# stdstu12/YUME

Hardware: AMD Instinct MI355X
Metric: denoise-steps/sec (Yume-5B 720P, 33-frame latent) (higher is better)
Workload: dtype bf16; 1 GPU; Yume-5B-720P random-init, 33-frame 704x1280 clip (latent 48x13x44x80, FramePack lfz=8, L=9460), ODE Euler steps of a 50-step shift-7 schedule, no CFG, one chain per GPU; num_layers=30, parallelism=dp1 (independent chains, replicated weights)

## Files before the change

yume_amd/csrc/gemm_f8.hpp:

```cpp
#pragma once
#include "gemm_w4.hpp"

namespace gemm_f8 {
using namespace gemm_core;

typedef __attribute__((ext_vector_type(8))) int i32x8;

constexpr int F8_BK = 128;
constexpr int F8_NTHR = 256;
constexpr int F8_OPER = 256 * F8_BK;
constexpr int F8_BUF = 2 * F8_OPER;
constexpr int F8_LDS = 2 * F8_BUF;

struct F8Args {
    const unsigned char* A; int64_t lda; const float* sa;
    const unsigned char* W; int64_t ldw; const float* sw;
    const unsigned char* ea; int64_t ldea;
    unsigned char* eo; int64_t ldeo;
};

constexpr int EPI_MX_GELU = YUME_EPI_MX_GELU;

__device__ __forceinline__ void f8_stage(const unsigned char* const (&ga)[8], const unsigned char* const (&gw)[8], int koff, char* buf, int wave) {
#pragma unroll
    for (int j = 0; j < 8; ++j)
        __builtin_amdgcn_global_load_lds((gbl_cvoid*)(ga[j] + koff), (lds_void*)(buf + j * 4096 + wave * 1024), 16, 0, 0);
#pragma unroll
    for (int j = 0; j < 8; ++j)
        __builtin_amdgcn_global_load_lds((gbl_cvoid*)(gw[j] + koff), (lds_void*)(buf + F8_OPER + j * 4096 + wave * 1024), 16, 0, 0);
}

__device__ __forceinline__ i32x8 f8_frag(const char* oper, int row, int lane) {
    const int q = lane >> 4;
    const char* rp = oper + row * F8_BK;
    const u32x4 lo = *reinterpret_cast<const u32x4*>(rp + ((((2 * q) ^ row) & 7) << 4));
    const u32x4 hi = *reinterpret_cast<const u32x4*>(rp + ((((2 * q + 1) ^ row) & 7) << 4));
    return i32x8{(int)lo[0], (int)lo[1], (int)lo[2], (int)lo[3], (int)hi[0], (int)hi[1], (int)hi[2], (int)hi[3]};
}

template <class Col>
__device__ __forceinline__ void f8_epilogue_vt(const f32x4 (&acc)[8][8], const float (&sa)[8], Col col, const Problem& p, const Epilogue& e, int m0,
                                               int n0, char* smem) {
    const int lane = threadIdx.x & 63;
    const int wave = __builtin_amdgcn_readfirstlane(threadIdx.x >> 6);
    const int wr = wave >> 1, wc = wave & 1;
    const int l15 = lane & 15, l4 = lane >> 4;
    const bool odd = (l15 & 1) != 0;
    const int x0 = 4 * l4 + 2 * (l15 & 1);
    const unsigned vbase = (unsigned)((wc * 128 + x0) * 512 + ((l15 >> 1) & 3) * 4);
    const unsigned lx = (unsigned)((x0 | (l15 >> 3)) << 4);
    __syncthreads();
#pragma unroll
    for (int j = 0; j < 8; ++j) {
        f32x4 sw, b;
        col(j, sw, b);
        const unsigned jb = vbase + (unsigned)(16 * j * 512) + (unsigned)((wr ^ (j & 1)) << 8);
#pragma unroll
        for (int i = 0; i < 8; ++i) {
            const f32x4 v = (acc[i][j] * sa[i]) * sw + b;
            const unsigned p01 = pack_bf16x2(v[0], v[1]), p23 = pack_bf16x2(v[2], v[3]);
            const unsigned got = (unsigned)__builtin_amdgcn_update_dpp(0, (int)(odd ? p01 : p23), 0xB1, 0xf, 0xf, false);
            const unsigned keep = odd ? p23 : p01;
            const unsigned lo = odd ? got : keep, hi = odd ? keep : got;
            *reinterpret_cast<unsigned*>(smem + jb + (lx ^ (unsigned)((2 * i) << 4))) = (lo & 0xffffu) | (hi << 16);
            *reinterpret_cast<unsigned*>(smem + jb + 512u + (lx ^ (unsigned)((2 * i + 1) << 4))) = (lo >> 16) | (hi & 0xffff0000u);
        }
    }
    __syncthreads();
    gemm_w4::w4_store_image(smem, e.outT + (int64_t)(n0 - e.n_split) * e.ldt, e.ldt, 0, min(256, p.N - n0), m0, min(256, p.M - m0));
}

template <int EPI, bool MX = false>
__device__ __forceinline__ void f8_epilogue(const f32x4 (&acc)[8][8], const Problem& p, const F8Args& f, const Epilogue& e, int m0, int n0, char* smem) {
    const int lane = threadIdx.x & 63;
    const int wave = __builtin_amdgcn_readfirstlane(threadIdx.x >> 6);
    const int wr = wave >> 1, wc = wave & 1;
    const int l15 = lane & 15, l4 = lane >> 4;
    float sa[8];
#pragma unroll
    for (int i = 0; i < 8; ++i) sa[i] = MX ? 1.0f : f.sa[min(m0 + wr * 128 + 16 * i + l15, p.M - 1)];
    auto col = [&](int j, f32x4& sw, f32x4& b) {
        const int n = n0 + wc * 128 + 16 * j + 4 * l4;
        sw = n < p.N ? *reinterpret_cast<const f32x4*>(f.sw + n) : f32x4{1.f, 1.f, 1.f, 1.f};
        b = (e.bias && n < p.N) ? *reinterpret_cast<const f32x4*>(e.bias + n) : f32x4{0.f, 0.f, 0.f, 0.f};
    };
    if constexpr (EPI == YUME_EPI_BF16_SPLITT) {
        if (n0 >= e.n_split) {
            f8_epilogue_vt(acc, sa, col, p, e, m0, n0, smem);
            return;
        }
    }
    constexpr int EPI_RM = EPI == YUME_EPI_BF16_SPLITT ? YUME_EPI_BF16 : EPI;
    constexpr bool BF16_OUT = EPI_RM == YUME_EPI_BF16 || EPI_RM == YUME_EPI_BF16_GELU;
    if (BF16_OUT && (e.ldo % 8) == 0) {
        const gemm_w4::ImageOff io = gemm_w4::w4_image_offsets(wr, wc, l15, l4);
        __syncthreads();
#pragma unroll
        for (int j = 0; j < 8; ++j) {
            f32x4 sw, b;
            col(j, sw, b);
#pragma unroll
            for (int i = 0; i < 8; ++i) {
                const f32x4 v = gemm_w4::w4_act<EPI>((acc[i][j] * sa[i]) * sw + b);
                u32x2 o;
                o[0] = pack_bf16x2(v[0], v[1]);
                o[1] = pack_bf16x2(v[2], v[3]);
                *reinterpret_cast<u32x2*>(smem + ((i & 1) ? io.o[j] : io.e[j]) + i * 8192) = o;
            }
        }
        __syncthreads();
        gemm_w4::w4_store_image(smem, reinterpret_cast<unsigned short*>(e.out), e.ldo, m0, min(256, p.M - m0), n0, min(256, p.N - n0));
        return;
    }
    Epilogue e0 = e;
    e0.bias = nullptr;
#pragma unroll
    for (int j = 0; j < 8; ++j) {
        f32x4 sw, b;
        col(j, sw, b);
#pragma unroll
        for (int i = 0; i < 8; ++i) {
            const int m = m0 + wr * 128 + 16 * i + l15, n = n0 + wc * 128 + 16 * j + 4 * l4;
            if (m < p.M && n < p.N) store_row4<EPI_RM>((acc[i][j] * sa[i]) * sw + b, m, n, p, e0);
        }
    }
}

__device__ __forceinline__ void f8_epilogue_mx_gelu(const f32x4 (&acc)[8][8], const Problem& p, const F8Args& f, const Epilogue& e, int m0, int n0) {
    const int lane = threadIdx.x & 63;
    const int wave = __builtin_amdgcn_readfirstlane(threadIdx.x >> 6);
    const int wr = wave >> 1, wc = wave & 1;
    const int l15 = lane & 15, l4 = lane >> 4;
    float sa[8];
#pragma unroll
    for (int i = 0; i < 8; ++i) sa[i] = f.sa[min(m0 + wr * 128 + 16 * i + l15, p.M - 1)];
    unsigned char* const qo = reinterpret_cast<unsigned char*>(e.out);
#pragma unroll
    for (int jj = 0; jj < 4; ++jj) {
        const int nb = n0 + wc * 128 + 32 * jj;
        const bool in_n = nb < p.N;
        f32x4 sw[2], b[2];
#pragma unroll
        for (int h = 0; h < 2; ++h) {
            const int n = nb + 16 * h + 4 * l4;
            sw[h] = in_n ? *reinterpret_cast<const f32x4*>(f.sw + n) : f32x4{1.f, 1.f, 1.f, 1.f};
            b[h] = (e.bias && in_n) ? *reinterpret_cast<const f32x4*>(e.bias + n) : f32x4{0.f, 0.f, 0.f, 0.f};
        }
#pragma unroll
        for (int i = 0; i < 8; ++i) {
            const int m = m0 + wr * 128 + 16 * i + l15;
            f32x4 v[2];
            float am = 0.f;
#pragma unroll
            for (int h = 0; h < 2; ++h) {
                v[h] = gemm_w4::w4_act<YUME_EPI_BF16_GELU>((acc[i][2 * jj + h] * sa[i]) * sw[h] + b[h]);
#pragma unroll
                for (int c = 0; c < 4; ++c) am = fmaxf(am, fabsf(v[h][c]));
            }
            am = fmaxf(am, __shfl_xor(am, 16, 64));
            am = fmaxf(am, __shfl_xor(am, 32, 64));
            const unsigned bits = __float_as_uint(am);
            const int E = (int)(bits >> 23);
            int byte = E - 8 + ((bits & 0x7fffffu) > 0x600000u ? 1 : 0);
            byte = am > 0.f ? max(byte, 0) : 127;
            const float mult = __uint_as_float((unsigned)(254 - byte) << 23);
            if (m < p.M && in_n) {
#pragma unroll
                for (int h = 0; h < 2; ++h) {
                    float t[4];
#pragma unroll
                    for (int c = 0; c < 4; ++c) t[c] = fminf(fmaxf(v[h][c] * mult, -448.0f), 448.0f);
                    int w = __builtin_amdgcn_cvt_pk_fp8_f32(t[0], t[1], 0, false);
                    w = __builtin_amdgcn_cvt_pk_fp8_f32(t[2], t[3], w, true);
                    *reinterpret_cast<int*>(qo + (int64_t)m * e.ldo + nb + 16 * h + 4 * l4) = w;
                }
                if (l4 == 0) f.eo[(int64_t)m * f.ldeo + (nb >> 5)] = (unsigned char)byte;
            }
        }
    }
}

__device__ __forceinline__ i32x8 f8_frag_mx(const char* oper, int row, int lane) {
    const int q = lane >> 4;
    const char* rp = oper + row * F8_BK;
    const u32x4 lo = *reinterpret_cast<const u32x4*>(rp + (((q ^ row) & 7) << 4));
    const u32x4 hi = *reinterpret_cast<const u32x4*>(rp + ((((4 + q) ^ row) & 7) << 4));
    return i32x8{(int)lo[0], (int)lo[1], (int)lo[2], (int)lo[3], (int)hi[0], (int)hi[1], (int)hi[2], (int)hi[3]};
}

__device__ __forceinline__ void f8_mx_scales_load(const unsigned char* const (&ge)[8], int g, u32x4 (&raw)[8]) {
#pragma unroll
    for (int i = 0; i < 8; ++i) raw[i] = *reinterpret_cast<const u32x4*>(ge[i] + 16 * g);
}
__device__ __forceinline__ void f8_mx_scales_pack(const u32x4 (&raw)[8], int lane, unsigned (&pk)[8]) {
    const int sh = 8 * (lane >> 4);
#pragma unroll
    for (int i = 0; i < 8; ++i)
        pk[i] = ((raw[i][0] >> sh) & 0xffu) | (((raw[i][1] >> sh) & 0xffu) << 8) | (((raw[i][2] >> sh) & 0xffu) << 16) | ((raw[i][3] >> sh) << 24 & 0xff000000u);
}

template <int EPI>
__global__ __launch_bounds__(F8_NTHR, 1) void gemm_f8_mx_kernel(Problem p, F8Args f, Epilogue e) {
    __shared__ __attribute__((aligned(16))) char smem[F8_LDS];
    const int tid = threadIdx.x;
    const int lane = tid & 63;
    const int wave = __builtin_amdgcn_readfirstlane(tid >> 6);
    const int wr = wave >> 1, wc = wave & 1;
    int start, count, m0, n0;
    xcd_chunk(p.tiles_m * p.tiles_n, blockIdx.x & 7, start, count);
    tile_origin(p, start + (blockIdx.x >> 3), m0, n0);

    const unsigned char* ga[8];
    const unsigned char* gw[8];
    const unsigned char* ge[8];
    {
        const int rl = 8 * wave + (lane >> 3);
#pragma unroll
        for (int j = 0; j < 8; ++j) {
            const int r = 32 * j + rl;
            const int ch = ((lane & 7) ^ (r & 7)) << 4;
            ga[j] = f.A + (int64_t)min(m0 + r, p.M - 1) * f.lda + ch;
            gw[j] = f.W + (int64_t)min(n0 + r, p.N - 1) * f.ldw + ch;
        }
#pragma unroll
        for (int i = 0; i < 8; ++i) ge[i] = f.ea + (int64_t)min(m0 + wr * 128 + 16 * i + (lane & 15), p.M - 1) * f.ldea;
    }
    f32x4 acc[8][8];
#pragma unroll
    for (int i = 0; i < 8; ++i)
#pragma unroll
        for (int j = 0; j < 8; ++j) acc[i][j] = f32x4{0.f, 0.f, 0.f, 0.f};

    const int nk = p.K / F8_BK;
    u32x4 raw[8];
    unsigned pk[8], pkn[8];
    f8_mx_scales_load(ge, 0, raw);
    f8_stage(ga, gw, 0, smem, wave);
    f8_mx_scales_pack(raw, lane, pk);
#pragma unroll
    for (int i = 0; i < 8; ++i) pkn[i] = pk[i];
    int cur = 0;
    for (int kt = 0; kt < nk; ++kt) {
        asm volatile("s_waitcnt vmcnt(0)" ::: "memory");
        __syncthreads();
        const int t = kt & 3;
        if (t == 3) f8_mx_scales_pack(raw, lane, pkn);
        if (t == 2 && kt + 2 < nk) f8_mx_scales_load(ge, (kt >> 2) + 1, raw);
        if (kt + 1 < nk) f8_stage(ga, gw, (kt + 1) * F8_BK, smem + (cur ^ 1) * F8_BUF, wave);
        const char* At = smem + cur * F8_BUF;
        const char* Wt = At + F8_OPER;
        i32x8 a[8];
        int sc[8];
#pragma unroll
        for (int i = 0; i < 8; ++i) {
            a[i] = f8_frag_mx(At, wr * 128 + 16 * i + (lane & 15), lane);
            sc[i] = (int)(pk[i] >> (8 * t));
        }
#pragma unroll
        for (int j = 0; j < 8; ++j) {
            const i32x8 w = f8_frag_mx(Wt, wc * 128 + 16 * j + (lane & 15), lane);
#pragma unroll
            for (int i = 0; i < 8; ++i)
                acc[i][j] = __builtin_amdgcn_mfma_scale_f32_16x16x128_f8f6f4(w, a[i], acc[i][j], 0, 0, 0, 0x7f7f7f7f, 0, sc[i]);
        }
        if (t == 3) {
#pragma unroll
            for (int i = 0; i < 8; ++i) pk[i] = pkn[i];
        }
        cur ^= 1;
    }
    f8_epilogue<EPI, true>(acc, p, f, e, m0, n0, smem);
}

template <int EPI>
__global__ __launch_bounds__(F8_NTHR, 1) void gemm_f8_kernel(Problem p, F8Args f, Epilogue e) {
    __shared__ __attribute__((aligned(16))) char smem[F8_LDS];
    const int tid = threadIdx.x;
    const int lane = tid & 63;
    const int wave = __builtin_amdgcn_readfirstlane(tid >> 6);
    const int wr = wave >> 1, wc = wave & 1;
    int start, count, m0, n0;
    xcd_chunk(p.tiles_m * p.tiles_n, blockIdx.x & 7, start, count);
    tile_origin(p, start + (blockIdx.x >> 3), m0, n0);

    const unsigned char* ga[8];
    const unsigned char* gw[8];
    {
        const int rl = 8 * wave + (lane >> 3);
#pragma unroll
        for (int j = 0; j < 8; ++j) {
            const int r = 32 * j + rl;
            const int ch = ((lane & 7) ^ (r & 7)) << 4;
            ga[j] = f.A + (int64_t)min(m0 + r, p.M - 1) * f.lda + ch;
            gw[j] = f.W + (int64_t)min(n0 + r, p.N - 1) * f.ldw + ch;
        }
    }
    f32x4 acc[8][8];
#pragma unroll
    for (int i = 0; i < 8; ++i)
#pragma unroll
        for (int j = 0; j < 8; ++j) acc[i][j] = f32x4{0.f, 0.f, 0.f, 0.f};

    const int nk = p.K / F8_BK;
    f8_stage(ga, gw, 0, smem, wave);
    int cur = 0;
    for (int kt = 0; kt < nk; ++kt) {
        asm volatile("s_waitcnt vmcnt(0)" ::: "memory");
        __syncthreads();
        if (kt + 1 < nk) f8_stage(ga, gw, (kt + 1) * F8_BK, smem + (cur ^ 1) * F8_BUF, wave);
        const char* At = smem + cur * F8_BUF;
        const char* Wt = At + F8_OPER;
        i32x8 a[8];
#pragma unroll
        for (int i = 0; i < 8; ++i) a[i] = f8_frag(At, wr * 128 + 16 * i + (lane & 15), lane);
#pragma unroll
        for (int j = 0; j < 8; ++j) {
            const i32x8 w = f8_frag(Wt, wc * 128 + 16 * j + (lane & 15), lane);
#pragma unroll
            for (int i = 0; i < 8; ++i)
                acc[i][j] = __builtin_amdgcn_mfma_scale_f32_16x16x128_f8f6f4(w, a[i], acc[i][j], 0, 0, 0, 0x7f7f7f7f, 0, 0x7f7f7f7f);
        }
        cur ^= 1;
    }
    if constexpr (EPI == EPI_MX_GELU) f8_epilogue_mx_gelu(acc, p, f, e, m0, n0);
    else f8_epilogue<EPI>(acc, p, f, e, m0, n0, smem);
}

inline int launch_f8(int epi, Problem p, const F8Args& f, const Epilogue& e, hipStream_t st) {
    p.tiles_m = (p.M + 255) / 256;
    p.tiles_n = (p.N + 255) / 256;
    p.group_m = g_group_m;
    const dim3 grid((unsigned)(p.tiles_m * p.tiles_n)), block(F8_NTHR);
    switch (epi) {
        case YUME_EPI_BF16_GELU: hipLaunchKernelGGL(gemm_f8_kernel<YUME_EPI_BF16_GELU>, grid, block, 0, st, p, f, e); break;
        case YUME_EPI_F32: hipLaunchKernelGGL(gemm_f8_kernel<YUME_EPI_F32>, grid, block, 0, st, p, f, e); break;
        case YUME_EPI_RESID: hipLaunchKernelGGL(gemm_f8_kernel<YUME_EPI_RESID>, grid, block, 0, st, p, f, e); break;
        case EPI_MX_GELU: hipLaunchKernelGGL(gemm_f8_kernel<EPI_MX_GELU>, grid, block, 0, st, p, f, e); break;
        case YUME_EPI_BF16_SPLITT: hipLaunchKernelGGL(gemm_f8_kernel<YUME_EPI_BF16_SPLITT>, grid, block, 0, st, p, f, e); break;
        default: hipLaunchKernelGGL(gemm_f8_kernel<YUME_EPI_BF16>, grid, block, 0, st, p, f, e); break;
    }
    YUME_CHECK_LAUNCH("gemm_f8");
    return YUME_OK;
}

inline int launch_f8_mx(int epi, Problem p, const F8Args& f, const Epilogue& e, hipStream_t st) {
    p.tiles_m = (p.M + 255) / 256;
    p.tiles_n = (p.N + 255) / 256;
    p.group_m = g_group_m;
    const dim3 grid((unsigned)(p.tiles_m * p.tiles_n)), block(F8_NTHR);
    if (epi == YUME_EPI_RESID) hipLaunchKernelGGL(gemm_f8_mx_kernel<YUME_EPI_RESID>, grid, block, 0, st, p, f, e);
    else hipLaunchKernelGGL(gemm_f8_mx_kernel<YUME_EPI_F32>, grid, block, 0, st, p, f, e);
    YUME_CHECK_LAUNCH("gemm_f8_mx");
    return YUME_OK;
}

}
```

Baseline: 10.46 denoise-steps/sec.

## Interleave FP8 GEMM LDS reads, global loads and MFMAs with sched group barriers

Adds a scheduled main-loop variant for the FP8 and MX-FP8 GEMM kernels. It uses sched_group_barrier to interleave LDS fragment reads and next-tile global loads between the 64 MFMAs of each K step, and peels the last iteration so it does no staging. The goal is to hide memory latency behind matrix work instead of letting the compiler cluster loads. The variant is on by default for the GELU, RESID and MX-GELU epilogues and selectable through an environment variable, at the cost of doubled template instantiations and more register pressure.

```diff
diff --git a/yume_amd/csrc/gemm_f8.hpp b/yume_amd/csrc/gemm_f8.hpp
--- a/yume_amd/csrc/gemm_f8.hpp
+++ b/yume_amd/csrc/gemm_f8.hpp
@@ -199,7 +199,41 @@
         pk[i] = ((raw[i][0] >> sh) & 0xffu) | (((raw[i][1] >> sh) & 0xffu) << 8) | (((raw[i][2] >> sh) & 0xffu) << 16) | ((raw[i][3] >> sh) << 24 & 0xff000000u);
 }
 
-template <int EPI>
+constexpr int F8_SG_MFMA = 0x8, F8_SG_VMEM = 0x10, F8_SG_DS_READ = 0x100;
+template <bool MX, bool STAGE>
+__device__ __forceinline__ void f8_tile_sched(f32x4 (&acc)[8][8], const char* __restrict__ At, const unsigned char* const (&ga)[8],
+                                              const unsigned char* const (&gw)[8], int koff, char* __restrict__ nbuf, int wave, int wr, int wc, int lane,
+                                              const int (&sc)[8]) {
+    __builtin_amdgcn_sched_barrier(0);
+    if constexpr (STAGE) f8_stage(ga, gw, koff, nbuf, wave);
+    const char* Wt = At + F8_OPER;
+    i32x8 a[8];
+#pragma unroll
+    for (int i = 0; i < 8; ++i) a[i] = MX ? f8_frag_mx(At, wr * 128 + 16 * i + (lane & 15), lane) : f8_frag(At, wr * 128 + 16 * i + (lane & 15), lane);
+#pragma unroll
+    for (int j = 0; j < 8; ++j) {
+        const i32x8 w = MX ? f8_frag_mx(Wt, wc * 128 + 16 * j + (lane & 15), lane) : f8_frag(Wt, wc * 128 + 16 * j + (lane & 15), lane);
+#pragma unroll
+        for (int i = 0; i < 8; ++i)
+            acc[i][j] = __builtin_amdgcn_mfma_scale_f32_16x16x128_f8f6f4(w, a[i], acc[i][j], 0, 0, 0, 0x7f7f7f7f, 0, MX ? sc[i] : 0x7f7f7f7f);
+    }
+    __builtin_amdgcn_sched_group_barrier(F8_SG_DS_READ, 8, 0);
+#pragma unroll
+    for (int m = 0; m < 64; ++m) {
+        __builtin_amdgcn_sched_group_barrier(F8_SG_MFMA, 1, 0);
+        if (m < 5 || m == 5 || (m >= 8 && m < 56 && (m & 7) == 3)) __builtin_amdgcn_sched_group_barrier(F8_SG_DS_READ, 2, 0);
+        if (STAGE && m < 32 && (m & 1)) __builtin_amdgcn_sched_group_barrier(F8_SG_VMEM, 1, 0);
+    }
+    __builtin_amdgcn_sched_barrier(0);
+    if constexpr (!STAGE) {
+#pragma unroll
+        for (int i = 0; i < 8; ++i)
+#pragma unroll
+            for (int j = 0; j < 8; ++j) asm volatile("" : "+a"(acc[i][j]));
+    }
+}
+
+template <int EPI, int LOOP>
 __global__ __launch_bounds__(F8_NTHR, 1) void gemm_f8_mx_kernel(Problem p, F8Args f, Epilogue e) {
     __shared__ __attribute__((aligned(16))) char smem[F8_LDS];
     const int tid = threadIdx.x;
@@ -240,6 +274,25 @@
 #pragma unroll
     for (int i = 0; i < 8; ++i) pkn[i] = pk[i];
     int cur = 0;
+    if constexpr (LOOP == 1) {
+        int sc[8];
+        for (int kt = 0; kt + 1 < nk; ++kt) {
+            asm volatile("s_waitcnt vmcnt(0)" ::: "memory");
+            __syncthreads();
+            const int t = kt & 3;
+#pragma unroll
+            for (int i = 0; i < 8; ++i) sc[i] = (int)(pk[i] >> (8 * t));
+            if (t == 3) f8_mx_scales_pack(raw, lane, pk);
+            if (t == 2 && kt + 2 < nk) f8_mx_scales_load(ge, (kt >> 2) + 1, raw);
+            f8_tile_sched<true, true>(acc, smem + cur * F8_BUF, ga, gw, (kt + 1) * F8_BK, smem + (cur ^ 1) * F8_BUF, wave, wr, wc, lane, sc);
+            cur ^= 1;
+        }
+        asm volatile("s_waitcnt vmcnt(0)" ::: "memory");
+        __syncthreads();
+#pragma unroll
+        for (int i = 0; i < 8; ++i) sc[i] = (int)(pk[i] >> (8 * ((nk - 1) & 3)));
+        f8_tile_sched<true, false>(acc, smem + cur * F8_BUF, ga, gw, 0, smem, wave, wr, wc, lane, sc);
+    } else
     for (int kt = 0; kt < nk; ++kt) {
         asm volatile("s_waitcnt vmcnt(0)" ::: "memory");
         __syncthreads();
@@ -272,7 +325,7 @@
     f8_epilogue<EPI, true>(acc, p, f, e, m0, n0, smem);
 }
 
-template <int EPI>
+template <int EPI, int LOOP>
 __global__ __launch_bounds__(F8_NTHR, 1) void gemm_f8_kernel(Problem p, F8Args f, Epilogue e) {
     __shared__ __attribute__((aligned(16))) char smem[F8_LDS];
     const int tid = threadIdx.x;
@@ -304,6 +357,18 @@
     const int nk = p.K / F8_BK;
     f8_stage(ga, gw, 0, smem, wave);
     int cur = 0;
+    if constexpr (LOOP == 1) {
+        const int sc[8] = {};
+        for (int kt = 0; kt + 1 < nk; ++kt) {
+            asm volatile("s_waitcnt vmcnt(0)" ::: "memory");
+            __syncthreads();
+            f8_tile_sched<false, true>(acc, smem + cur * F8_BUF, ga, gw, (kt + 1) * F8_BK, smem + (cur ^ 1) * F8_BUF, wave, wr, wc, lane, sc);
+            cur ^= 1;
+        }
+        asm volatile("s_waitcnt vmcnt(0)" ::: "memory");
+        __syncthreads();
+        f8_tile_sched<false, false>(acc, smem + cur * F8_BUF, ga, gw, 0, smem, wave, wr, wc, lane, sc);
+    } else
     for (int kt = 0; kt < nk; ++kt) {
         asm volatile("s_waitcnt vmcnt(0)" ::: "memory");
         __syncthreads();
@@ -325,6 +390,16 @@
     if constexpr (EPI == EPI_MX_GELU) f8_epilogue_mx_gelu(acc, p, f, e, m0, n0);
     else f8_epilogue<EPI>(acc, p, f, e, m0, n0, smem);
 }
+
+inline bool f8_loop_sched(bool dflt) {
+    static const int env = [] { const char* v = getenv("YUME_GEMM_F8_LOOP"); return v ? (atoi(v) != 0 ? 1 : 0) : -1; }();
+    return env < 0 ? dflt : env != 0;
+}
+#define F8_LAUNCH(KERNEL, EPI_, DFLT)                                                                              \
+    do {                                                                                                           \
+        if (f8_loop_sched(DFLT)) hipLaunchKernelGGL((KERNEL<EPI_, 1>), grid, block, 0, st, p, f, e);               \
+        else hipLaunchKernelGGL((KERNEL<EPI_, 0>), grid, block, 0, st, p, f, e);                                   \
+    } while (0)
 
 inline int launch_f8(int epi, Problem p, const F8Args& f, const Epilogue& e, hipStream_t st) {
     p.tiles_m = (p.M + 255) / 256;
@@ -332,12 +407,12 @@
     p.group_m = g_group_m;
     const dim3 grid((unsigned)(p.tiles_m * p.tiles_n)), block(F8_NTHR);
     switch (epi) {
-        case YUME_EPI_BF16_GELU: hipLaunchKernelGGL(gemm_f8_kernel<YUME_EPI_BF16_GELU>, grid, block, 0, st, p, f, e); break;
-        case YUME_EPI_F32: hipLaunchKernelGGL(gemm_f8_kernel<YUME_EPI_F32>, grid, block, 0, st, p, f, e); break;
-        case YUME_EPI_RESID: hipLaunchKernelGGL(gemm_f8_kernel<YUME_EPI_RESID>, grid, block, 0, st, p, f, e); break;
-        case EPI_MX_GELU: hipLaunchKernelGGL(gemm_f8_kernel<EPI_MX_GELU>, grid, block, 0, st, p, f, e); break;
-        case YUME_EPI_BF16_SPLITT: hipLaunchKernelGGL(gemm_f8_kernel<YUME_EPI_BF16_SPLITT>, grid, block, 0, st, p, f, e); break;
-        default: hipLaunchKernelGGL(gemm_f8_kernel<YUME_EPI_BF16>, grid, block, 0, st, p, f, e); break;
+        case YUME_EPI_BF16_GELU: F8_LAUNCH(gemm_f8_kernel, YUME_EPI_BF16_GELU, true); break;
+        case YUME_EPI_F32: F8_LAUNCH(gemm_f8_kernel, YUME_EPI_F32, false); break;
+        case YUME_EPI_RESID: F8_LAUNCH(gemm_f8_kernel, YUME_EPI_RESID, true); break;
+        case EPI_MX_GELU: F8_LAUNCH(gemm_f8_kernel, EPI_MX_GELU, true); break;
+        case YUME_EPI_BF16_SPLITT: F8_LAUNCH(gemm_f8_kernel, YUME_EPI_BF16_SPLITT, false); break;
+        default: F8_LAUNCH(gemm_f8_kernel, YUME_EPI_BF16, false); break;
     }
     YUME_CHECK_LAUNCH("gemm_f8");
     return YUME_OK;
@@ -348,10 +423,11 @@
     p.tiles_n = (p.N + 255) / 256;
     p.group_m = g_group_m;
     const dim3 grid((unsigned)(p.tiles_m * p.tiles_n)), block(F8_NTHR);
-    if (epi == YUME_EPI_RESID) hipLaunchKernelGGL(gemm_f8_mx_kernel<YUME_EPI_RESID>, grid, block, 0, st, p, f, e);
-    else hipLaunchKernelGGL(gemm_f8_mx_kernel<YUME_EPI_F32>, grid, block, 0, st, p, f, e);
+    if (epi == YUME_EPI_RESID) F8_LAUNCH(gemm_f8_mx_kernel, YUME_EPI_RESID, true);
+    else F8_LAUNCH(gemm_f8_mx_kernel, YUME_EPI_F32, false);
     YUME_CHECK_LAUNCH("gemm_f8_mx");
     return YUME_OK;
 }
-
-}
+#undef F8_LAUNCH
+
+}
```

Result: no change. 10.42 denoise-steps/sec (-0.4%).
